# nvlong21/Lightweight-face-detection-CenterNet

Measured on AMD Instinct MI355X. Metric: images/sec at 640x640 batch inference, higher is better.
Workload: dtype bf16; 1 GPU; BASELINE configs[1]: batch=64 640x640 bf16 on 1 MI355X per rank, forward + top-100 peak decode; synthetic uint8 images resident in HBM, calibrated synthetic weights (seed 0); 2 context(s) per GPU, batch k on context k mod 2; batch_per_gpu=64, global_batch=64, topk=100, parallelism=dp1, contexts_per_gpu=2, input_buffers=4

## Files before the change

lightweight-face-detection-centernet_amd/csrc/cf_mbconv3.hip:

```cpp
#include "cf_exp.h"
#include "cf_common.h"
#include "cf_kernels.h"
#include "cf_mx.h"
#include <cstdlib>

namespace cf {

template <int KS, int JX, int TOH, int TOW, int NW, bool ALDS = true>
struct Mx {
    static constexpr int HC = 32;
    static constexpr int IH = TOH + KS - 1, IWQ = TOW / 4 + 1, IWP = IWQ * 4;
    static constexpr int NQD = IH * IWQ, NIB = (NQD + 7) / 8, IPX = NQD * 4;
    static constexpr int CP = HC * 8 + 16;
    static constexpr int EBYTES = NIB * 8 * CP;
    static constexpr int NOQ = TOH * (TOW / 4), NSET = (NOQ + 15) / 16;
    static constexpr int WXB = JX * 1024;
    static constexpr int NSTEP = KS * 2;
    static constexpr int ATB = 2 * NSTEP * 512;
    static constexpr int LDS = EBYTES + WXB + (ALDS ? ATB : 0);
    static_assert(TOW % 4 == 0 && KS <= 5, "x-quads; two k-steps cover 4 + KS - 1 <= 8 inputs");
};

template <int KS, int JX, int TOH, int TOW, int NW, bool ALDS>
__global__ __launch_bounds__(NW * 64) void expdw_mx_kernel(MbParams p) {
    typedef Mx<KS, JX, TOH, TOW, NW, ALDS> G;
    constexpr int IWQ = G::IWQ, IWP = G::IWP, IPX = G::IPX, NIB = G::NIB, CP = G::CP, NSET = G::NSET, WXB = G::WXB;
    extern __shared__ __attribute__((aligned(16))) char smem[];
    char* E = smem;
    char* Wst = smem + G::EBYTES;

    const int tid = threadIdx.x, lane = tid & 63;
    const int wave = __builtin_amdgcn_readfirstlane(tid >> 6);
    const int pl = lane & 31, h = lane >> 5;
    const int tiles_x = (p.Wout + TOW - 1) / TOW;
    const int tyi = blockIdx.x / tiles_x, txi = blockIdx.x - tyi * tiles_x;
    const int ox0 = txi * TOW, oy0 = tyi * TOH, b = blockIdx.z;
    const int grp = blockIdx.y;

    {
        const char* srcx = (const char*)p.wexp + (size_t)grp * WXB;
        for (int c = wave; c < WXB / 1024; c += NW)
            __builtin_amdgcn_global_load_lds((const __attribute__((address_space(1))) void*)(srcx + c * 1024 + lane * 16),
                                             (__attribute__((address_space(3))) void*)(Wst + c * 1024), 16, 0, 0);
    }
    asm volatile("" ::: "memory");
    char* Ats = Wst + WXB;
    u32x2 A[ALDS ? 1 : 2][ALDS ? 1 : KS][2];
    if constexpr (ALDS) {
        const char* srca = (const char*)p.wdw + (size_t)grp * G::ATB;
        for (int c = wave; c < G::ATB / 1024; c += NW)
            __builtin_amdgcn_global_load_lds((const __attribute__((address_space(1))) void*)(srca + c * 1024 + lane * 16),
                                             (__attribute__((address_space(3))) void*)(Ats + c * 1024), 16, 0, 0);
    } else {
        const u32x2* at = reinterpret_cast<const u32x2*>(p.wdw) + (size_t)grp * (2 * KS * 2) * 64 + lane;
#pragma unroll
        for (int q = 0; q < 2; ++q)
#pragma unroll
            for (int ky = 0; ky < KS; ++ky)
#pragma unroll
                for (int ks = 0; ks < 2; ++ks) A[q][ky][ks] = at[((q * KS + ky) * 2 + ks) * 64];
    }
    asm volatile("" ::: "memory");
    const char* xbase = (const char*)p.x + (size_t)b * p.Hin * p.Win * p.Cin * 2;
    const unsigned rowbytes = (unsigned)p.Cin * 2;
    auto load_x = [&](int ib, u32x4* xf) -> bool {
        const int ip = ib * 32 + pl;
        const int ipc = ip < IPX ? ip : IPX - 1;
        const int iy = ipc / IWP, ix = ipc - iy * IWP;
        const int gy = oy0 - p.pad_lo + iy, gx = ox0 - p.pad_lo + ix;
        const int cy = min(max(gy, 0), p.Hin - 1), cx = min(max(gx, 0), p.Win - 1);
        if (p.xblock) {
            const char* xb = (const char*)p.x + blk_off(((size_t)b * p.Hin + cy) * p.Win + cx, p.Cin / 8, h * JX);
#pragma unroll
            for (int j = 0; j < JX; ++j) xf[j] = ld16(xb + j * 512);
        } else {
            const unsigned off = ((unsigned)cy * (unsigned)p.Win + (unsigned)cx) * rowbytes + (unsigned)(h * JX * 16);
#pragma unroll
            for (int j = 0; j < JX; ++j) xf[j] = ld16(xbase + off + j * 16);
        }
        return ip < IPX && (unsigned)gy < (unsigned)p.Hin && (unsigned)gx < (unsigned)p.Win;
    };
    const bool last_in = (h * JX + JX - 1) * 8 < p.Cin;
    auto mask_x = [&](u32x4* xf, bool valid) {
#pragma unroll
        for (int j = 0; j < JX; ++j) {
            const bool vj = j == JX - 1 ? (valid && last_in) : valid;
            xf[j].x = vj ? xf[j].x : 0u; xf[j].y = vj ? xf[j].y : 0u; xf[j].z = vj ? xf[j].z : 0u; xf[j].w = vj ? xf[j].w : 0u;
        }
    };
#ifdef CF_ABLATION
    const int abl = p.nw;
#else
    constexpr int abl = 0;
#endif
    u32x4 xa[JX];
    bool va = false;
    if (wave < NIB) va = load_x(wave, xa);
    static_assert(NIB >= NW, "every wave issues the X loads the wait below keeps in flight");
    cf_sync_lds_dma_keep<(ALDS ? 0 : 2 * KS * 2) + JX>();
    mask_x(xa, va);

    for (int ib = wave; ib < NIB; ib += NW) {
        u32x4 xn[JX];
        const bool more = ib + NW < NIB;
        bool vn = false;
        if (more) { if (abl & 8) { for (int j = 0; j < JX; ++j) xn[j] = xa[j]; vn = va; } else vn = load_x(ib + NW, xn); }
        f32x16 a;
#pragma unroll
        for (int r = 0; r < 16; ++r) a[r] = 0.0f;
        const char* wb = Wst + lane * 16;
#pragma unroll
        for (int j = 0; j < JX; ++j) {
            const u32x4 wv = ld16(wb + j * 1024);
            a = __builtin_amdgcn_mfma_f32_32x32x16_bf16(__builtin_bit_cast(mfma_bf16x8, xa[j]),
                                                        __builtin_bit_cast(mfma_bf16x8, wv), a, 0, 0, 0);
        }
        char* ecell = E + (unsigned)(ib * 8 + h) * (unsigned)CP + pl * 8;
#pragma unroll
        for (int t = 0; t < 4; ++t) {
            f32x2 u0, u1; u0.x = a[4 * t]; u0.y = a[4 * t + 1]; u1.x = a[4 * t + 2]; u1.y = a[4 * t + 3];
            f32x2 y0 = u0, y1 = u1;
            if (!(abl & 4)) { y0 = swish2_pre(u0); y1 = swish2_pre(u1); }
            u32x2 d;
            d.x = __builtin_bit_cast(uint32_t, __builtin_amdgcn_cvt_pkrtz(y0.x, y0.y));
            d.y = __builtin_bit_cast(uint32_t, __builtin_amdgcn_cvt_pkrtz(y1.x, y1.y));
            *reinterpret_cast<u32x2*>(ecell + 2 * t * CP) = d;
        }
        if (more) {
#pragma unroll
            for (int j = 0; j < JX; ++j) xa[j] = xn[j];
            mask_x(xa, vn);
        }
    }
    __syncthreads();

    static constexpr SetMap<TOH, TOW, IWQ> kSets{};
    const int kg = lane >> 4;
    for (int set = wave; set < NSET; set += NW) {
        const uint32_t e = kSets.v[set * 16 + (lane & 15)];
        const int oy = (e >> 6) & 0x1ff, oxq = e & 63;
        const bool live = (e & 0x8000u) == 0;
        f32x4 acc[8];
        const char* bb = E + (unsigned)(oy * IWQ + oxq) * (unsigned)CP + kg * 64;
        if (abl & 1) {
#pragma unroll
            for (int g = 0; g < 8; ++g) acc[g] = f32x4{(float)oy, (float)oxq, (float)g, 1.0f};
        } else {
        if constexpr (ALDS) mx_depthwise_lds<KS, IWQ, CP>(bb, Ats + lane * 8, acc);
        else mx_depthwise<KS, IWQ, CP>(bb, reinterpret_cast<const u32x2 (*)[KS][2]>(A), acc);
        }
        if (!(abl & 2))
#pragma unroll
        for (int g = 0; g < 8; ++g)
#pragma unroll
            for (int i = 0; i < 4; i += 2) {
                f32x2 u; u.x = acc[g][i]; u.y = acc[g][i + 1];
                const f32x2 y = swish2_pre(u) * kNegLn23;
                acc[g][i] = y.x; acc[g][i + 1] = y.y;
            }
        const int gy = oy0 + oy, gx0 = ox0 + 4 * oxq;
        if (!live || gy >= p.Hout || ((abl & 16) && acc[0][0] != 123.0f)) continue;
        const size_t opix0 = ((size_t)b * p.Hout + gy) * p.Wout + gx0;
        const int chunk = grp * 4 + kg;
#pragma unroll
        for (int i = 0; i < 4; ++i) {
            if (gx0 + i >= p.Wout) break;
            u32x4 o;
            o.x = packb(acc[0][i], acc[1][i]); o.y = packb(acc[2][i], acc[3][i]);
            o.z = packb(acc[4][i], acc[5][i]); o.w = packb(acc[6][i], acc[7][i]);
            const size_t opix = opix0 + i;
            if (abl & 32) {
                const size_t region = (((size_t)b * gridDim.x + blockIdx.x) * gridDim.y + grp) * (size_t)(TOH * TOW * 64);
                st16((char*)p.y + region + ((size_t)((set * 4 + i) * 1024 + lane * 16)) % (size_t)(TOH * TOW * 64), o);
                continue;
            }
            st16((char*)p.y + (p.yblock ? blk_off(opix, p.hid / 8, chunk) : (opix * p.hid + (size_t)chunk * 8) * 2), o);
        }
    }
}

#include CF_EXP_INC(cf_mbconv3_0)

template <int KS, int JX, int NMB, int TOH, int TOW, int NW, bool TAIL16, bool ALDS = false>
struct Fx {
    static constexpr int IH = TOH + KS - 1, IWQ = TOW / 4 + 1, IWP = IWQ * 4;
    static constexpr int NQD = IH * IWQ, NIB = (NQD + 7) / 8, IPX = NQD * 4, MAXI = (NIB + NW - 1) / NW;
    static constexpr int CP8 = 32 * 8 + 16, CP4 = 16 * 8 + 16;
    static constexpr int EBYTES = NIB * 8 * CP8;
    static constexpr int NOQ = TOH * (TOW / 4), NSET = (NOQ + 15) / 16, SPW = NSET / NW;
    static constexpr int WXB = JX * 1024;
    static constexpr int ATB = 2 * KS * 2 * 512;
    static constexpr int LDS = EBYTES + 2 * WXB + (ALDS ? ATB : 0);
    static_assert(NSET % NW == 0, "every wave owns SPW whole sets (project accumulators live in registers)");
    static_assert(TOW % 4 == 0 && KS <= 5 && (NMB == 2 || NMB == 4 || NMB == 6), "geometry");
    static_assert(!TAIL16 || JX <= 2, "16-channel round: one 16x16x32 expand MFMA, Cin <= 32");
};

template <int KS, int JX, int NMB, bool RESID, int TOH, int TOW, int NW, bool TAIL16, bool XRELOAD, bool ALDS, bool SB = false>
__global__ __launch_bounds__(NW * 64) void mbconv_mx_kernel(MbParams p) {
    typedef Fx<KS, JX, NMB, TOH, TOW, NW, TAIL16, ALDS> G;
    constexpr int IWQ = G::IWQ, IWP = G::IWP, IPX = G::IPX, NIB = G::NIB, MAXI = G::MAXI, CP8 = G::CP8, CP4 = G::CP4;
    constexpr int SPW = G::SPW, WXB = G::WXB;
    extern __shared__ __attribute__((aligned(16))) char smem[];
    char* E = smem;
    char* Wst = smem + G::EBYTES;
    char* Ats = Wst + 2 * G::WXB;

    const int tid = threadIdx.x, lane = tid & 63;
    const int wave = __builtin_amdgcn_readfirstlane(tid >> 6);
    const int pl = lane & 31, h = lane >> 5, kg = lane >> 4;
    const int ox0 = blockIdx.x * TOW, oy0 = blockIdx.y * TOH, b = blockIdx.z;
    const int nq = p.nq;
#ifdef CF_ABLATION
    const int abl = p.nw;
#else
    constexpr int abl = 0;
#endif

    const char* xbase = (const char*)p.x + (size_t)b * p.Hin * p.Win * p.Cin * 2;
    const unsigned rowbytes = (unsigned)p.Cin * 2;

    auto stage_weights = [&](int q) {
        char* dst = Wst + (q & 1) * WXB;
        const char* srcx = (const char*)p.wexp + (size_t)q * WXB;
        for (int c = wave; c < WXB / 1024; c += NW)
            __builtin_amdgcn_global_load_lds((const __attribute__((address_space(1))) void*)(srcx + c * 1024 + lane * 16),
                                             (__attribute__((address_space(3))) void*)(dst + c * 1024), 16, 0, 0);
    };

    u32x4 xf[MAXI][JX];
    auto load_x = [&]() {
#pragma unroll
    for (int t = 0; t < MAXI; ++t) {
        const int ib = wave + NW * t;
        const int ip = ib * 32 + pl;
        const int ipc = ip < IPX ? ip : IPX - 1;
        const int iy = ipc / IWP, ix = ipc - iy * IWP;
        const int gy = oy0 - p.pad_lo + iy, gx = ox0 - p.pad_lo + ix;
        const bool valid = ip < IPX && (unsigned)gy < (unsigned)p.Hin && (unsigned)gx < (unsigned)p.Win;
        const int cy = min(max(gy, 0), p.Hin - 1), cx = min(max(gx, 0), p.Win - 1);
        const unsigned off = ((unsigned)cy * (unsigned)p.Win + (unsigned)cx) * rowbytes + (unsigned)(h * JX * 16);
#pragma unroll
        for (int j = 0; j < JX; ++j) {
            const bool vj = valid && (h * JX + j) * 8 < p.Cin;
            const u32x4 v = ld16(xbase + off + j * 16);
            xf[t][j].x = vj ? v.x : 0u; xf[t][j].y = vj ? v.y : 0u;
            xf[t][j].z = vj ? v.z : 0u; xf[t][j].w = vj ? v.w : 0u;
        }
    }
    };
    if constexpr (!XRELOAD) load_x();

    static constexpr SetMap<TOH, TOW, IWQ> kSets{};
    unsigned qcell[SPW];
#pragma unroll
    for (int sw = 0; sw < SPW; ++sw) {
        const uint32_t e = kSets.v[(wave * SPW + sw) * 16 + (lane & 15)];
        qcell[sw] = ((e >> 6) & 0x1ff) * IWQ + (e & 63);
    }
// ... 390 lines not shown
        __syncthreads();
        if (half == 0) {
            const char* bb = E + qcell * (unsigned)CP4 + kg * 32;
            f32x4 acc[4];
#pragma unroll
            for (int g = 0; g < 4; ++g) acc[g] = f32x4{0.0f, 0.0f, 0.0f, 0.0f};
#pragma unroll
            for (int st = 0; st < NSTEP; ++st) {
                const char* bs = bb + ((st / KSTEPS) * IWQ + ((st % KSTEPS) & 1) * HQ + ((st % KSTEPS) >> 1)) * CP4;
                const u32x4 b0 = ld16(bs), b1 = ld16(bs + 16);
                const mfma_f16x4 av = __builtin_bit_cast(mfma_f16x4, A4[st / KSTEPS][st % KSTEPS]);
                u32x2 t0, t1, t2, t3; t0.x = b0.x; t0.y = b0.y; t1.x = b0.z; t1.y = b0.w; t2.x = b1.x; t2.y = b1.y; t3.x = b1.z; t3.y = b1.w;
                CF_MX_MFMA(acc[0], av, __builtin_bit_cast(mfma_f16x4, t0), 0);
                CF_MX_MFMA(acc[1], av, __builtin_bit_cast(mfma_f16x4, t1), 1);
                CF_MX_MFMA(acc[2], av, __builtin_bit_cast(mfma_f16x4, t2), 2);
                CF_MX_MFMA(acc[3], av, __builtin_bit_cast(mfma_f16x4, t3), 3);
            }
#pragma unroll
            for (int g = 0; g < 4; ++g)
#pragma unroll
                for (int i = 0; i < 4; i += 2) {
                    f32x2 u; u.x = acc[g][i]; u.y = acc[g][i + 1];
                    const f32x2 y = swish2_pre(u);
                    acc[g][i] = y.x; acc[g][i + 1] = y.y;
                }
#pragma unroll
            for (int i = 0; i < 4; ++i) {
                u32x2 d; d.x = packb(acc[0][i], acc[1][i]); d.y = packb(acc[2][i], acc[3][i]);
#pragma unroll
                for (int mb = 0; mb < NMB; ++mb)
                    pacc[i][mb] = __builtin_amdgcn_mfma_f32_16x16x16bf16_1k(__builtin_bit_cast(mfma_bf16x4, wp4[mb]),
                                                                            __builtin_bit_cast(mfma_bf16x4, d), pacc[i][mb], 0, 0, 0);
            }
        }
    }

    __syncthreads();
    {
        f32x4* red = reinterpret_cast<f32x4*>(smem) + ((size_t)set * 64 + lane) * (4 * NMB);
        if (half == 1) {
#pragma unroll
            for (int i = 0; i < 4; ++i)
#pragma unroll
                for (int mb = 0; mb < NMB; ++mb) red[i * NMB + mb] = pacc[i][mb];
        }
        __syncthreads();
        if (half == 1) return;
#pragma unroll
        for (int i = 0; i < 4; ++i)
#pragma unroll
            for (int mb = 0; mb < NMB; ++mb) pacc[i][mb] += red[i * NMB + mb];
    }
    const int gy = oy0 + soy, gx0 = ox0 + 4 * soxq;
    if ((se & 0x8000u) || gy >= p.Hout) return;
    const size_t opix0 = ((size_t)b * p.Hout + gy) * p.Wout + gx0;
#pragma unroll
    for (int i = 0; i < 4; ++i) {
        if (gx0 + i >= p.Wout) break;
        const size_t opix = opix0 + i;
#pragma unroll
        for (int mp = 0; mp < NMB / 2; ++mp) {
            const int ch = mp * 32 + kg * 8;
            if (ch >= p.Cout) break;
            float v[8];
#pragma unroll
            for (int r = 0; r < 4; ++r) { v[r] = pacc[i][2 * mp][r]; v[4 + r] = pacc[i][2 * mp + 1][r]; }
            st16((char*)p.y + (p.yblock ? blk_off(opix, p.Cout / 8, ch / 8) : (opix * p.Cout + ch) * 2), pack16b(v));
        }
    }
}
#ifndef CF_ILP_TU

struct MxEntry {
    int k, jx, toh, tow, nw, var, lds_bytes;
    hipError_t (*fn)(hipStream_t, const MbParams&);
};
template <int KS, int JX, int TOH, int TOW, int NW, bool ALDS>
static hipError_t xmx_launch_t(hipStream_t s, const MbParams& p) {
    typedef Mx<KS, JX, TOH, TOW, NW, ALDS> G;
    dim3 grid(((p.Wout + TOW - 1) / TOW) * ((p.Hout + TOH - 1) / TOH), p.hid / 32, p.B), blk(NW * 64);
    set_kernel_tag("void cf::expdw_mx_kernel<%d, %d, %d, %d, %d, %s>(cf::MbParams)", KS, JX, TOH, TOW, NW, ALDS ? "true" : "false");
    static const int abl = cf_ab_int("CF_MX_ABL", 0);
    MbParams q = p; q.nw = abl;
    return launch_lds<expdw_mx_kernel<KS, JX, TOH, TOW, NW, ALDS>>(grid, blk, G::LDS, s, q);
}
#include CF_EXP_INC(cf_mbconv3_2)
#include CF_EXP_INC(cf_mbconv3_3)
#define XMT(V, KS, JX, TOH, TOW, NW, T) {KS, JX, TOH, TOW, NW, V, Mx<KS, JX, TOH, TOW, NW, true>::LDS, &xmxt_launch_t<KS, JX, TOH, TOW, NW, T>}
#define XMR(V, KS, JX, TOH, TOW, NW, R) {KS, JX, TOH, TOW, NW, V, Mx<KS, JX, TOH, TOW, NW, true>::EBYTES + 2 * (Mx<KS, JX, TOH, TOW, NW, true>::WXB + Mx<KS, JX, TOH, TOW, NW, true>::ATB), &xmxr_launch_t<KS, JX, TOH, TOW, NW, R>}
#define XMX(V, KS, JX, TOH, TOW, NW, AL) {KS, JX, TOH, TOW, NW, V, Mx<KS, JX, TOH, TOW, NW, (AL != 0)>::LDS, &xmx_launch_t<KS, JX, TOH, TOW, NW, (AL != 0)>}
static const MxEntry kXmxTable[] = {
    XMX(0, 5, 4, 10, 40, 8, 1),
    XMX(0, 5, 6, 10, 40, 8, 1),
    XMX(0, 5, 10, 20, 20, 4, 0),
    XMX(0, 3, 10, 10, 20, 4, 1),
#include CF_EXP_INC(cf_mbconv3_4)
};
#undef XMT
#undef XMX
#undef XMR
static const MxEntry* xmx_find(int k, int jx) {
    static const int want = cf_ab_int("CF_MX_VARIANT", 0);
    return pick_variant(kXmxTable, want, [&](const MxEntry& e) { return e.k == k && e.jx == jx; });
}

MbGeom expdw_mx_geometry(int dtype, int Cin, int hid, int k, int s) {
    MbGeom g{};
    static const bool off = cf_env_int("CF_DW_MATRIX", 1) == 0 || cf_ab_int("CF_MX", 1) == 0;
    if (off || dtype != 1 || s != 1 || (Cin % 8) || (hid % 32) || hid == Cin) return g;
    const int jx = (Cin * 2 / 16 + 1) / 2;
    const MxEntry* e = xmx_find(k, jx);
    if (!e) return g;
    g.ok = true; g.kind = XD_MX; g.S = 1;
    g.JX = jx; g.NBO = 0; g.HC = 32; g.nq = hid / 32; g.NBE = 1; g.HALF = 0;
    g.rowb = 32 * 8 + 16;
    g.lds_bytes = (size_t)e->lds_bytes;
    g.wexp_bytes = (size_t)g.nq * g.JX * 64 * 16;
    g.wdw_floats = (size_t)g.nq * 2 * k * 2 * 64 * 2;
    g.wproj_bytes = 0;
    return g;
}

void mx_pack_taps(int nq, int k, const float* wd , uint32_t* out, int stride, int ksteps) {
    for (int r = 0; r < nq; ++r)
        for (int q = 0; q < 2; ++q)
            for (int ky = 0; ky < k; ++ky)
                for (int ks = 0; ks < ksteps; ++ks)
                    for (int lane = 0; lane < 64; ++lane) {
                        const int kg = lane >> 4, pg = (lane >> 2) & 3, i = lane & 3;
                        const float* wrow = wd + (size_t)(r * 32 + kg * 8 + q * 4 + pg) * k * k + (size_t)ky * k;
                        uint16_t v[4];
                        for (int kk = 0; kk < 4; ++kk) {
                            const int kx = 4 * ks + kk - stride * i;
                            v[kk] = (kx >= 0 && kx < k) ? host_f32_to_f16_3(wrow[kx]) : 0;
                        }
                        uint32_t* dst = out + ((((size_t)(r * 2 + q) * k + ky) * ksteps + ks) * 64 + lane) * 2;
                        dst[0] = (uint32_t)v[0] | ((uint32_t)v[1] << 16);
                        dst[1] = (uint32_t)v[2] | ((uint32_t)v[3] << 16);
                    }
}

void mx_pack_weights(int, const MbGeom& g, int Cin, int hid, int Cout, int k, const float* we, const float* wd, const float* wp,
                     void* wexp_host, float* wdw_host, void* wproj_host) {
    (void)hid; (void)Cout; (void)wp; (void)wproj_host;
    const int NCx = Cin * 2 / 16;
    __builtin_memset(wexp_host, 0, g.wexp_bytes);
    for (int q = 0; q < g.nq; ++q)
        for (int j = 0; j < g.JX; ++j)
            for (int lane = 0; lane < 64; ++lane) {
                const int n = lane & 31, hh = lane >> 5, c = hh * g.JX + j;
                if (c >= NCx) continue;
                uint16_t* dst = (uint16_t*)((char*)wexp_host + (((size_t)q * g.JX + j) * 64 + lane) * 16);
                for (int e = 0; e < 8; ++e) dst[e] = host_f32_to_bf16(kNegLog2e3 * we[(size_t)(q * 32 + n) * Cin + (size_t)c * 8 + e]);
            }
    mx_pack_taps(g.nq, k, wd, reinterpret_cast<uint32_t*>(wdw_host));
}

hipError_t mx_launch(hipStream_t s, int, const MbParams& p) {
    const MxEntry* e = xmx_find(p.k, p.JX);
    if (!e || p.s != 1) return hipErrorInvalidValue;
    return e->fn(s, p);
}


#endif
struct FxEntry {
    int k, jx, nmb, res, tail, toh, tow, nw, var, lds_bytes;
// ... 232 lines not shown
```

lightweight-face-detection-centernet_amd/csrc/cf_pw.hip:

```cpp
#include "cf_common.h"
#include "cf_kernels.h"
#include <cstdlib>
#include <type_traits>

namespace cf {

typedef __attribute__((ext_vector_type(8))) __bf16 mfma_bf16x8;

static inline int slot_channel(int nb, int i) {
    int h = (i >> 2) & 1;
    int r = (i & 3) + 4 * (i >> 3);
    return nb * 32 + h * 16 + r;
}

static inline int pw_chunks(int dtype, int K) { return (int)((size_t)K * elem_size(dtype) / 16); }

size_t pw_packed_bytes(int dtype, int K, int N) {
    int NC = pw_chunks(dtype, K), NCh = (NC + 1) / 2;
    int NB = (N + 31) / 32;
    int NBpad = (NB + 7) / 8 * 8;
    return (size_t)NBpad * NCh * 64 * 16;
}

void pw_pack_weights(int dtype, const float* w, int K, int N, void* out_host) {
// ... 51 lines not shown
        u32x4 xc[4], wc[4][NBW];
#pragma unroll
        for (int u = 0; u < 4; ++u) {
            const int j = j0 + u < NCh ? j0 + u : NCh - 1;
            xc[u] = ld16(xrow + (size_t)(j < jmax ? j : 0) * xs);
#pragma unroll
            for (int i = 0; i < NBW; ++i)
                wc[u][i] = ld16(wbase + ((size_t)(i < nbv ? i : 0) * NCh + j) * 1024);
        }
        if constexpr (std::is_same<T, sp32_t>::value) {
#pragma unroll
            for (int u = 0; u < 4; u += 2) {
                if (j0 + u + 1 < NCh) {
#pragma unroll
                    for (int i = 0; i < NBW; ++i)
                        if (i < nbv) Mma<T>::run2(acc[i], wc[u][i], wc[u + 1][i], xc[u], xc[u + 1]);
                } else if (j0 + u < NCh) {
#pragma unroll
                    for (int i = 0; i < NBW; ++i)
                        if (i < nbv) Mma<T>::run(acc[i], wc[u][i], xc[u]);
                }
            }
        } else {
#pragma unroll
        for (int u = 0; u < 4; ++u) {
            if (j0 + u < NCh) {
#pragma unroll
                for (int i = 0; i < NBW; ++i)
                    if (i < nbv) Mma<T>::run(acc[i], wc[u][i], xc[u]);
            }
        }
        }
    }

    if (!mvalid) return;
    size_t low_row = 0; int tap = 0;
    if constexpr (RES == 2) {
        long long hw = (long long)p.Ho * p.Wo;
        long long b = m / hw; int rem = (int)(m - b * hw);
        int yy = rem / p.Wo, xx = rem - yy * p.Wo;
        low_row = ((size_t)b * (p.Ho >> 1) + (yy >> 1)) * (p.Wo >> 1) + (xx >> 1);
        tap = ((yy & 1) << 1) | (xx & 1);
    }
#pragma unroll
    for (int i = 0; i < NBW; ++i) {
        if (nb0 + i >= NB) break;
        const int cb = (nb0 + i) * 32 + h * 16;
#pragma unroll
        for (int g = 0; g < 16 / P; ++g) {
            const int ch = cb + g * P;
            if (ch >= p.N) break;
            float v[P];
#pragma unroll
            for (int e = 0; e < P; ++e) {
                float t = acc[i][g * P + e];
                if constexpr (BIAS) t += p.bias[ch + e];
                v[e] = t;
            }
            act_arr<ACT, P>(v);
            if constexpr (RES == 1) {
                float r[P];
                unpack16<T>(ld16((const char*)p.res + (p.resblock ? blk_off((size_t)m, p.N / P, ch / P) : ((size_t)m * p.N + ch) * sizeof(T))), r);
#pragma unroll
                for (int e = 0; e < P; ++e) v[e] += r[e];
            } else if constexpr (RES == 2) {
                float r[P];
                unpack16<T>(ld16((const char*)p.low + (low_row * p.N + ch) * sizeof(T)), r);
#pragma unroll
                for (int e = 0; e < P; ++e)
                    v[e] += relu_f(r[e] * p.upw[tap * p.N + ch + e] + p.upb[ch + e]);
            }
            const size_t ld = p.ldy ? (size_t)p.ldy : (size_t)p.N;
            st16((char*)p.y + (p.yblock ? blk_off((size_t)m, p.N / P, ch / P) : ((size_t)m * ld + p.yoff + ch) * sizeof(T)), pack16<T>(v));
        }
    }
}

template <typename T, int NBW, int ACT, int RES, int NST>
__global__ __launch_bounds__(256) void pw_wlds_kernel(PwParams p) {
    constexpr int P = Elem<T>::PER16;
    constexpr int KT = 4;
    extern __shared__ __attribute__((aligned(16))) char smem[];
    const int lane = threadIdx.x & 63;
    const int wave = threadIdx.x >> 6;
    const int pl = lane & 31, h = lane >> 5;
    const long long pb = (long long)blockIdx.x * 4 + wave;
    const long long m = pb * 32 + pl;
    const bool mvalid = m < p.M;
    const long long mr = mvalid ? m : p.M - 1;
    const int NC = (int)((size_t)p.K * sizeof(T) / 16), NCh = (NC + 1) >> 1;
    const int NB = (p.N + 31) >> 5;
    const int nb0 = blockIdx.y * NBW;
    const size_t xs = p.xblock ? 512 : 16;
    const long long pbc = pb * 32 < p.M ? pb : (p.M - 1) / 32;
    const char* xrow = p.xblock ? (const char*)p.x + (((size_t)pbc * NC + (size_t)h * NCh) * 32 + pl) * 16
                                : (const char*)p.x + (size_t)mr * p.K * sizeof(T) + (size_t)h * NCh * 16;
    const int jmax = (h == 0) ? NCh : NC - NCh;

    f32x16 acc[NBW];
#pragma unroll
    for (int i = 0; i < NBW; ++i)
#pragma unroll
        for (int r = 0; r < 16; ++r) acc[i][r] = 0.0f;

    constexpr int STAGE = NBW * KT * 1024;
    constexpr int VM_PER_TILE = NBW * KT / 4 + KT;
    const int NT = (NCh + KT - 1) / KT;
    auto prefetch = [&](int t, char* stage, u32x4* xn) {
        const int j0 = t * KT;
#pragma unroll
        for (int q = 0; q < NBW * KT / 4; ++q) {
            const int c = wave + 4 * q;
            const int i = c / KT, jj = c - i * KT;
            const int ii = nb0 + i < NB ? nb0 + i : NB - 1, jc = j0 + jj < NCh ? j0 + jj : NCh - 1;
            const char* src = (const char*)p.wp + ((((size_t)ii * NCh + jc) * 64) + lane) * 16;
            __builtin_amdgcn_global_load_lds((const __attribute__((address_space(1))) void*)src,
                                             (__attribute__((address_space(3))) void*)(stage + (i * KT + jj) * 1024), 16, 0, 0);
        }
#pragma unroll
        for (int jj = 0; jj < KT; ++jj) xn[jj] = ld16(xrow + (size_t)(j0 + jj < jmax ? j0 + jj : 0) * xs);
    };
    const int nbv = NB - nb0 < NBW ? NB - nb0 : NBW;
    u32x4 xr[NST][KT];
#pragma unroll
    for (int s0 = 0; s0 < NST - 1; ++s0)
        if (s0 < NT) prefetch(s0, smem + s0 * STAGE, xr[s0]);
    for (int t0 = 0; t0 < NT; t0 += NST) {
#pragma unroll
        for (int u = 0; u < NST; ++u) {
            const int t = t0 + u;
            if (t >= NT) break;
            const int younger = min(NT - 1 - t, NST - 2);
            if (NST >= 4 && younger >= 2) __builtin_amdgcn_s_waitcnt(((2 * VM_PER_TILE) & 0xF) | (((2 * VM_PER_TILE) >> 4) << 14) | 0x0F70);
            else if (NST >= 3 && younger >= 1) __builtin_amdgcn_s_waitcnt((VM_PER_TILE & 0xF) | ((VM_PER_TILE >> 4) << 14) | 0x0F70);
            else __builtin_amdgcn_s_waitcnt(0x0F70);
            __builtin_amdgcn_s_barrier();
            if (t + NST - 1 < NT) prefetch(t + NST - 1, smem + ((u + NST - 1) % NST) * STAGE, xr[(u + NST - 1) % NST]);
            const int kt = NCh - t * KT < KT ? NCh - t * KT : KT;
            const char* st = smem + u * STAGE;
            if constexpr (std::is_same<T, sp32_t>::value) {
#pragma unroll
                for (int jj = 0; jj < KT; jj += 2) {
                    if (jj + 1 < kt) {
#pragma unroll
                        for (int i = 0; i < NBW; ++i)
                            if (i < nbv) Mma<T>::run2(acc[i], ld16(st + (i * KT + jj) * 1024 + lane * 16), ld16(st + (i * KT + jj + 1) * 1024 + lane * 16),
                                                      xr[u][jj], xr[u][jj + 1]);
                    } else if (jj < kt) {
#pragma unroll
                        for (int i = 0; i < NBW; ++i)
                            if (i < nbv) Mma<T>::run(acc[i], ld16(st + (i * KT + jj) * 1024 + lane * 16), xr[u][jj]);
                    }
                }
            } else if (nbv == NBW) {
#pragma unroll
                for (int jj = 0; jj < KT; ++jj) {
                    if (jj < kt) {
#pragma unroll
                        for (int i = 0; i < NBW; ++i) Mma<T>::run(acc[i], ld16(st + (i * KT + jj) * 1024 + lane * 16), xr[u][jj]);
                    }
                }
            } else {
#pragma unroll
                for (int jj = 0; jj < KT; ++jj) {
                    if (jj < kt) {
#pragma unroll
                        for (int i = 0; i < NBW; ++i)
                            if (i < nbv) Mma<T>::run(acc[i], ld16(st + (i * KT + jj) * 1024 + lane * 16), xr[u][jj]);
                    }
                }
            }
        }
    }
    if (!mvalid) return;
#pragma unroll
    for (int i = 0; i < NBW; ++i) {
        if (nb0 + i >= NB) break;
        const int cb = (nb0 + i) * 32 + h * 16;
#pragma unroll
        for (int g = 0; g < 16 / P; ++g) {
            const int ch = cb + g * P;
            if (ch >= p.N) break;
            float v[P];
#pragma unroll
            for (int e = 0; e < P; ++e) v[e] = acc[i][g * P + e];
            act_arr<ACT, P>(v);
            if constexpr (RES == 1) {
                float r[P];
                unpack16<T>(ld16((const char*)p.res + (p.resblock ? blk_off((size_t)m, p.N / P, ch / P) : ((size_t)m * p.N + ch) * sizeof(T))), r);
#pragma unroll
                for (int e = 0; e < P; ++e) v[e] += r[e];
            }
            st16((char*)p.y + (p.yblock ? blk_off((size_t)m, p.N / P, ch / P) : ((size_t)m * p.N + ch) * sizeof(T)), pack16<T>(v));
        }
    }
}

template <int NBW, int ACT, int RES>
__global__ __launch_bounds__(256) void pw_ksplit_kernel(PwParams p) {
    typedef bf16_t T;
    constexpr int DEPTH = 4;
    extern __shared__ __attribute__((aligned(16))) char smem[];
    const int lane = threadIdx.x & 63;
    const int wave = __builtin_amdgcn_readfirstlane(threadIdx.x >> 6);
    const int pl = lane & 31, h = lane >> 5;
    const long long pb = blockIdx.x;
    const long long m = pb * 32 + pl;
    const bool mvalid = m < p.M;
    const long long mr = mvalid ? m : p.M - 1;
    const int NC = (int)((size_t)p.K * sizeof(T) / 16), NCh = (NC + 1) >> 1;
    const int NB = (p.N + 31) >> 5;
    const int nb0 = blockIdx.y * NBW;
    const size_t xs = p.xblock ? 512 : 16;
    const char* xrow = p.xblock ? (const char*)p.x + (((size_t)pb * NC + (size_t)h * NCh) * 32 + pl) * 16
                                : (const char*)p.x + (size_t)mr * p.K * sizeof(T) + (size_t)h * NCh * 16;
    const int jmax = (h == 0) ? NCh : NC - NCh;
    const int per = (NCh + 3) >> 2;
    const int j0 = wave * per, j1 = min(j0 + per, NCh);
    size_t woff[NBW];
#pragma unroll
    for (int i = 0; i < NBW; ++i) woff[i] = ((size_t)min(nb0 + i, NB - 1) * NCh * 64 + lane) * 16;

    f32x16 acc[NBW];
#pragma unroll
    for (int i = 0; i < NBW; ++i)
#pragma unroll
        for (int r = 0; r < 16; ++r) acc[i][r] = 0.0f;

    u32x4 xr[DEPTH], wr[DEPTH][NBW];
    auto fetch = [&](int j, int slot) {
        xr[slot] = ld16(xrow + (size_t)(j < jmax ? j : 0) * xs);
#pragma unroll
        for (int i = 0; i < NBW; ++i) wr[slot][i] = ld16((const char*)p.wp + woff[i] + (size_t)j * 1024);
    };
#pragma unroll
    for (int d = 0; d < DEPTH - 1; ++d)
        if (j0 + d < j1) fetch(j0 + d, d);
    for (int jb = j0; jb < j1; jb += DEPTH) {
#pragma unroll
        for (int u = 0; u < DEPTH; ++u) {
            const int j = jb + u;
            if (j >= j1) break;
            if (j + DEPTH - 1 < j1) fetch(j + DEPTH - 1, (u + DEPTH - 1) % DEPTH);
#pragma unroll
            for (int i = 0; i < NBW; ++i) Mma<T>::run(acc[i], wr[u][i], xr[u]);
        }
    }
    {
        f32x4* red = reinterpret_cast<f32x4*>(smem);
#pragma unroll
        for (int i = 0; i < NBW; ++i)
#pragma unroll
            for (int q = 0; q < 4; ++q) {
                f32x4 v; v[0] = acc[i][4 * q]; v[1] = acc[i][4 * q + 1]; v[2] = acc[i][4 * q + 2]; v[3] = acc[i][4 * q + 3];
                red[((wave * NBW + i) * 4 + q) * 64 + lane] = v;
            }
// ... 141 lines not shown
```

Baseline: 53260 images/s.

## Specialize expand-depthwise kernel for 32-bit addressing and simplify pointwise loads

```diff
diff --git a/lightweight-face-detection-centernet_amd/csrc/cf_mbconv3.hip b/lightweight-face-detection-centernet_amd/csrc/cf_mbconv3.hip
--- a/lightweight-face-detection-centernet_amd/csrc/cf_mbconv3.hip
+++ b/lightweight-face-detection-centernet_amd/csrc/cf_mbconv3.hip
@@ -21,8 +21,12 @@
     static_assert(TOW % 4 == 0 && KS <= 5, "x-quads; two k-steps cover 4 + KS - 1 <= 8 inputs");
 };
 
-template <int KS, int JX, int TOH, int TOW, int NW, bool ALDS>
+static __device__ __attribute__((aligned(16))) uint32_t kXmxZeros[10 * 512 / 4];
+
+template <int KS, int JX, int TOH, int TOW, int NW, bool ALDS, int MODE = 0>
 __global__ __launch_bounds__(NW * 64) void expdw_mx_kernel(MbParams p) {
+    constexpr bool FAST = MODE != 0, XB = FAST && ((MODE - 1) & 1), YB = FAST && ((MODE - 1) & 2), ODD = FAST && ((MODE - 1) & 4);
+    static_assert(JX <= 10, "kXmxZeros");
     typedef Mx<KS, JX, TOH, TOW, NW, ALDS> G;
     constexpr int IWQ = G::IWQ, IWP = G::IWP, IPX = G::IPX, NIB = G::NIB, CP = G::CP, NSET = G::NSET, WXB = G::WXB;
     extern __shared__ __attribute__((aligned(16))) char smem[];
@@ -63,8 +67,27 @@
     asm volatile("" ::: "memory");
     const char* xbase = (const char*)p.x + (size_t)b * p.Hin * p.Win * p.Cin * 2;
     const unsigned rowbytes = (unsigned)p.Cin * 2;
+    const int gy0 = oy0 - p.pad_lo, gx0h = ox0 - p.pad_lo;
+    const unsigned pix00 = ((unsigned)b * (unsigned)p.Hin + (unsigned)gy0) * (unsigned)p.Win;
+    const unsigned lanec = (unsigned)(h * JX) * (XB ? 512u : 16u);
+    const unsigned blkrow = (unsigned)(p.Cin / 8) * 512u;
+    typedef const __attribute__((address_space(1))) char* gptr_t;
+    gptr_t zeros = (gptr_t)kXmxZeros;
+    asm volatile("" : "+s"(zeros));
+    const unsigned hlim = (unsigned)min(p.Hin, gy0 + G::IH);
     auto load_x = [&](int ib, u32x4* xf) -> bool {
         const int ip = ib * 32 + pl;
+        if constexpr (FAST) {
+            const int iy = ip / IWP, ix = ip - iy * IWP;
+            const int gy = gy0 + iy, gx = gx0h + ix;
+            const bool valid = (unsigned)gy < hlim && (unsigned)gx < (unsigned)p.Win;
+            const unsigned pix = __umul24((unsigned)iy, (unsigned)p.Win) + (unsigned)gx + pix00;
+            const unsigned off = XB ? __umul24(pix >> 5, blkrow) + ((pix & 31u) << 4) + lanec : __umul24(pix, rowbytes) + lanec;
+            gptr_t xb = valid ? (gptr_t)p.x + off : zeros;
+#pragma unroll
+            for (int j = 0; j < JX; ++j) xf[j] = *(const __attribute__((address_space(1))) u32x4*)(xb + j * (XB ? 512 : 16));
+            return valid;
+        } else {
         const int ipc = ip < IPX ? ip : IPX - 1;
         const int iy = ipc / IWP, ix = ipc - iy * IWP;
         const int gy = oy0 - p.pad_lo + iy, gx = ox0 - p.pad_lo + ix;
@@ -79,13 +102,21 @@
             for (int j = 0; j < JX; ++j) xf[j] = ld16(xbase + off + j * 16);
         }
         return ip < IPX && (unsigned)gy < (unsigned)p.Hin && (unsigned)gx < (unsigned)p.Win;
+        }
     };
     const bool last_in = (h * JX + JX - 1) * 8 < p.Cin;
     auto mask_x = [&](u32x4* xf, bool valid) {
+        if constexpr (FAST) {
+            if constexpr (ODD) {
+                u32x4& v = xf[JX - 1];
+                v.x = h ? 0u : v.x; v.y = h ? 0u : v.y; v.z = h ? 0u : v.z; v.w = h ? 0u : v.w;
+            }
+        } else {
 #pragma unroll
         for (int j = 0; j < JX; ++j) {
             const bool vj = j == JX - 1 ? (valid && last_in) : valid;
             xf[j].x = vj ? xf[j].x : 0u; xf[j].y = vj ? xf[j].y : 0u; xf[j].z = vj ? xf[j].z : 0u; xf[j].w = vj ? xf[j].w : 0u;
+        }
         }
     };
 #ifdef CF_ABLATION
@@ -93,16 +124,21 @@
 #else
     constexpr int abl = 0;
 #endif
-    u32x4 xa[JX];
+    constexpr int MAXI = (NIB + NW - 1) / NW;
+    u32x4 xq[2][JX];
     bool va = false;
-    if (wave < NIB) va = load_x(wave, xa);
+    if (wave < NIB) va = load_x(wave, xq[0]);
     static_assert(NIB >= NW, "every wave issues the X loads the wait below keeps in flight");
     cf_sync_lds_dma_keep<(ALDS ? 0 : 2 * KS * 2) + JX>();
-    mask_x(xa, va);
-
-    for (int ib = wave; ib < NIB; ib += NW) {
-        u32x4 xn[JX];
-        const bool more = ib + NW < NIB;
+    mask_x(xq[0], va);
+
+#pragma unroll
+    for (int it = 0; it < MAXI; ++it) {
+        const int ib = wave + NW * it;
+        if (ib >= NIB) break;
+        u32x4* xa = xq[it & 1];
+        u32x4* xn = xq[(it + 1) & 1];
+        const bool more = it + 1 < MAXI && ib + NW < NIB;
         bool vn = false;
         if (more) { if (abl & 8) { for (int j = 0; j < JX; ++j) xn[j] = xa[j]; vn = va; } else vn = load_x(ib + NW, xn); }
         f32x16 a;
@@ -126,11 +162,7 @@
             d.y = __builtin_bit_cast(uint32_t, __builtin_amdgcn_cvt_pkrtz(y1.x, y1.y));
             *reinterpret_cast<u32x2*>(ecell + 2 * t * CP) = d;
         }
-        if (more) {
-#pragma unroll
-            for (int j = 0; j < JX; ++j) xa[j] = xn[j];
-            mask_x(xa, vn);
-        }
+        if (more) mask_x(xn, vn);
     }
     __syncthreads();
 
@@ -160,8 +192,36 @@
             }
         const int gy = oy0 + oy, gx0 = ox0 + 4 * oxq;
         if (!live || gy >= p.Hout || ((abl & 16) && acc[0][0] != 123.0f)) continue;
+        const int chunk = grp * 4 + kg;
+        if constexpr (FAST) {
+            if (gx0 >= p.Wout) continue;
+            const bool q4 = (p.Wout & 3) == 0;
+            const unsigned opix0 = __umul24((unsigned)b * (unsigned)p.Hout + (unsigned)gy, (unsigned)p.Wout) + (unsigned)gx0;
+            const unsigned yrow = (unsigned)p.hid * 2u, yblk = (unsigned)(p.hid / 8) * 512u;
+            char* yb = (char*)p.y;
+            if (YB && q4) {
+                const unsigned off = __umul24(opix0 >> 5, yblk) + ((opix0 & 31u) << 4) + (unsigned)chunk * 512u;
+#pragma unroll
+                for (int i = 0; i < 4; ++i) {
+                    u32x4 o;
+                    o.x = packb(acc[0][i], acc[1][i]); o.y = packb(acc[2][i], acc[3][i]);
+                    o.z = packb(acc[4][i], acc[5][i]); o.w = packb(acc[6][i], acc[7][i]);
+                    st16(yb + off + 16 * i, o);
+                }
+            } else {
+                const unsigned off0 = YB ? (unsigned)chunk * 512u : __umul24(opix0, yrow) + (unsigned)chunk * 16u;
+#pragma unroll
+                for (int i = 0; i < 4; ++i) {
+                    if (!q4 && gx0 + i >= p.Wout) break;
+                    u32x4 o;
+                    o.x = packb(acc[0][i], acc[1][i]); o.y = packb(acc[2][i], acc[3][i]);
+                    o.z = packb(acc[4][i], acc[5][i]); o.w = packb(acc[6][i], acc[7][i]);
+                    const unsigned opix = opix0 + i;
+                    st16(yb + (YB ? off0 + __umul24(opix >> 5, yblk) + ((opix & 31u) << 4) : off0 + (unsigned)i * yrow), o);
+                }
+            }
+        } else {
         const size_t opix0 = ((size_t)b * p.Hout + gy) * p.Wout + gx0;
-        const int chunk = grp * 4 + kg;
 #pragma unroll
         for (int i = 0; i < 4; ++i) {
             if (gx0 + i >= p.Wout) break;
@@ -175,6 +235,7 @@
                 continue;
             }
             st16((char*)p.y + (p.yblock ? blk_off(opix, p.hid / 8, chunk) : (opix * p.hid + (size_t)chunk * 8) * 2), o);
+        }
         }
     }
 }
@@ -731,7 +792,16 @@
     set_kernel_tag("void cf::expdw_mx_kernel<%d, %d, %d, %d, %d, %s>(cf::MbParams)", KS, JX, TOH, TOW, NW, ALDS ? "true" : "false");
     static const int abl = cf_ab_int("CF_MX_ABL", 0);
     MbParams q = p; q.nw = abl;
-    return launch_lds<expdw_mx_kernel<KS, JX, TOH, TOW, NW, ALDS>>(grid, blk, G::LDS, s, q);
+    const size_t mx = ((size_t)p.B * p.Hin * p.Win + 31) & ~(size_t)31, my = ((size_t)p.B * p.Hout * p.Wout + 31) & ~(size_t)31;
+    const bool small = abl == 0 && mx < ((size_t)1 << 24) && my < ((size_t)1 << 24) && mx * p.Cin * 2 + 16 < ((size_t)1 << 32) &&
+                       my * p.hid * 2 < ((size_t)1 << 32) && (size_t)p.Win < ((size_t)1 << 20);
+    if (!small) return launch_lds<expdw_mx_kernel<KS, JX, TOH, TOW, NW, ALDS, 0>>(grid, blk, G::LDS, s, q);
+    switch ((p.xblock ? 1 : 0) + (p.yblock ? 2 : 0) + ((p.Cin & 8) ? 4 : 0)) {
+#define CF_XMX_MODE(M) case M: return launch_lds<expdw_mx_kernel<KS, JX, TOH, TOW, NW, ALDS, M + 1>>(grid, blk, G::LDS, s, q);
+    CF_XMX_MODE(0) CF_XMX_MODE(1) CF_XMX_MODE(2) CF_XMX_MODE(3) CF_XMX_MODE(4) CF_XMX_MODE(5) CF_XMX_MODE(6) CF_XMX_MODE(7)
+#undef CF_XMX_MODE
+    }
+    return hipErrorInvalidValue;
 }
 #include CF_EXP_INC(cf_mbconv3_2)
 #include CF_EXP_INC(cf_mbconv3_3)
diff --git a/lightweight-face-detection-centernet_amd/csrc/cf_pw.hip b/lightweight-face-detection-centernet_amd/csrc/cf_pw.hip
--- a/lightweight-face-detection-centernet_amd/csrc/cf_pw.hip
+++ b/lightweight-face-detection-centernet_amd/csrc/cf_pw.hip
@@ -157,7 +157,7 @@
     constexpr int KT = 4;
     extern __shared__ __attribute__((aligned(16))) char smem[];
     const int lane = threadIdx.x & 63;
-    const int wave = threadIdx.x >> 6;
+    const int wave = __builtin_amdgcn_readfirstlane(threadIdx.x >> 6);
     const int pl = lane & 31, h = lane >> 5;
     const long long pb = (long long)blockIdx.x * 4 + wave;
     const long long m = pb * 32 + pl;
@@ -185,21 +185,34 @@
         const int j0 = t * KT;
 #pragma unroll
         for (int q = 0; q < NBW * KT / 4; ++q) {
-            const int c = wave + 4 * q;
-            const int i = c / KT, jj = c - i * KT;
+            static_assert(KT == 4, "fragment c = wave + 4 q of the tile is (n-block q, k-step wave)");
+            const int i = q, jj = wave;
             const int ii = nb0 + i < NB ? nb0 + i : NB - 1, jc = j0 + jj < NCh ? j0 + jj : NCh - 1;
-            const char* src = (const char*)p.wp + ((((size_t)ii * NCh + jc) * 64) + lane) * 16;
+            const char* src = (const char*)p.wp + (((size_t)ii * NCh + jc) * 64) * 16 + lane * 16;
             __builtin_amdgcn_global_load_lds((const __attribute__((address_space(1))) void*)src,
                                              (__attribute__((address_space(3))) void*)(stage + (i * KT + jj) * 1024), 16, 0, 0);
         }
-#pragma unroll
-        for (int jj = 0; jj < KT; ++jj) xn[jj] = ld16(xrow + (size_t)(j0 + jj < jmax ? j0 + jj : 0) * xs);
+        if (j0 + KT <= NC - NCh) {
+            const char* xt = xrow + (size_t)j0 * xs;
+            if (p.xblock) {
+#pragma unroll
+                for (int jj = 0; jj < KT; ++jj) xn[jj] = ld16(xt + jj * 512);
+            } else {
+#pragma unroll
+                for (int jj = 0; jj < KT; ++jj) xn[jj] = ld16(xt + jj * 16);
+            }
+        } else {
+#pragma unroll
+            for (int jj = 0; jj < KT; ++jj) xn[jj] = ld16(xrow + (size_t)(j0 + jj < jmax ? j0 + jj : 0) * xs);
+        }
     };
     const int nbv = NB - nb0 < NBW ? NB - nb0 : NBW;
     u32x4 xr[NST][KT];
 #pragma unroll
     for (int s0 = 0; s0 < NST - 1; ++s0)
         if (s0 < NT) prefetch(s0, smem + s0 * STAGE, xr[s0]);
+    auto kloop = [&](auto allnb) {
+    constexpr bool ALLNB = decltype(allnb)::value;
     for (int t0 = 0; t0 < NT; t0 += NST) {
 #pragma unroll
         for (int u = 0; u < NST; ++u) {
@@ -219,20 +232,12 @@
                     if (jj + 1 < kt) {
 #pragma unroll
                         for (int i = 0; i < NBW; ++i)
-                            if (i < nbv) Mma<T>::run2(acc[i], ld16(st + (i * KT + jj) * 1024 + lane * 16), ld16(st + (i * KT + jj + 1) * 1024 + lane * 16),
-                                                      xr[u][jj], xr[u][jj + 1]);
+                            if (ALLNB || i < nbv) Mma<T>::run2(acc[i], ld16(st + (i * KT + jj) * 1024 + lane * 16), ld16(st + (i * KT + jj + 1) * 1024 + lane * 16),
+                                                               xr[u][jj], xr[u][jj + 1]);
                     } else if (jj < kt) {
 #pragma unroll
                         for (int i = 0; i < NBW; ++i)
-                            if (i < nbv) Mma<T>::run(acc[i], ld16(st + (i * KT + jj) * 1024 + lane * 16), xr[u][jj]);
-                    }
-                }
-            } else if (nbv == NBW) {
-#pragma unroll
-                for (int jj = 0; jj < KT; ++jj) {
-                    if (jj < kt) {
-#pragma unroll
-                        for (int i = 0; i < NBW; ++i) Mma<T>::run(acc[i], ld16(st + (i * KT + jj) * 1024 + lane * 16), xr[u][jj]);
+                            if (ALLNB || i < nbv) Mma<T>::run(acc[i], ld16(st + (i * KT + jj) * 1024 + lane * 16), xr[u][jj]);
                     }
                 }
             } else {
@@ -241,12 +246,14 @@
                     if (jj < kt) {
 #pragma unroll
                         for (int i = 0; i < NBW; ++i)
-                            if (i < nbv) Mma<T>::run(acc[i], ld16(st + (i * KT + jj) * 1024 + lane * 16), xr[u][jj]);
+                            if (ALLNB || i < nbv) Mma<T>::run(acc[i], ld16(st + (i * KT + jj) * 1024 + lane * 16), xr[u][jj]);
                     }
                 }
             }
         }
     }
+    };
+    if (nbv == NBW) kloop(std::true_type{}); else kloop(std::false_type{});
     if (!mvalid) return;
 #pragma unroll
     for (int i = 0; i < NBW; ++i) {
```

New measurement: 53970 images/s, median of 6. 1.3% higher.
